# noahchalifour/rnnt-speech-recognition

Measured on AMD Instinct MI355X. Metric: rnnt_loss_grad_lattice_cells_per_sec, higher is better.
Workload: dtype f32

## Files before the change

rnnt-speech-recognition_amd/csrc/rnnt_common.h:

```cpp
#pragma once
#include <hip/hip_runtime.h>
#include <stdint.h>

#include <type_traits>

namespace rnnt {

constexpr float kNeg = -1.0e30f;
constexpr float kNegTest = -1.0e29f;
constexpr float kLog2e = 1.4426950408889634f;
constexpr float kLn2 = 0.6931471805599453f;
constexpr int kRebase = 8;

struct FastDiv {
    uint32_t d, m, s;
};
inline FastDiv make_fastdiv(uint32_t d) {
    FastDiv f;
    f.d = d;
    uint32_t s = 0;
    while ((1ull << s) < d) ++s;
    f.s = s;
    f.m = (uint32_t)((((1ull << s) - d) << 32) / d) + 1u;
    return f;
}
__device__ __forceinline__ uint32_t fdiv(uint32_t n, const FastDiv f) {
    return (__umulhi(n, f.m) + n) >> f.s;
}

struct TileGeom {
    int TT, UU, tiles_t, tiles_u, cpr;
    FastDiv div_tu, div_tt, divUU, div_cpr, divTT;
};

struct LossParams {
    const float *acts;
    float *grads;
    const int *labels;
    const int *label_lengths;
    const int *input_lengths;
    const float *cost_scale;
    float *costs;
    float *lse;
    float *W;
    float *A;
    float *Bt;
    float *offA;
    float *offB;
    double *ll;
    int *EA;
    int *EB;
    float *lik;
    int *flags;
    int NCl;
    float2 *pstat;
    int *lshift;
    int *bar;
    int nPstat;
    int pstatStride;
    int B, T, U, V, blank;
    int b0, nb;
    int visit_all;
    int precise;
    int N, Nr, Up, NC, NG;
    uint32_t cells;
    FastDiv divU, divT, divV, divOG;
    TileGeom tile;
};

struct WsLayout {
    size_t lse, W, A, Bt, offA, offB, ll, EA, EB, lik, flags, pstat, lshift, bar, total;
    int NCl, nPstat;
    int N, Nr, Up, NC, NG, OG;
};

inline size_t align_up(size_t x, size_t a) { return (x + a - 1) / a * a; }

constexpr int kMaxU = 8192;
inline int sweep_K(int U) {
    const int k = (U + 63) / 64;
    const int avail[] = {1, 2, 3, 4, 6, 8, 12, 16};
    for (int a : avail)
        if (k <= a) return a;
    return 0;
}
template <int K, int G>
struct SweepRing {
    static constexpr size_t kChunk = (size_t)G * 2 * 64 * K * sizeof(float);
    static constexpr int NB = (4 * kChunk + 16 <= 128 * 1024) ? 4 : 3;
    static constexpr size_t kBytes = NB * kChunk + 16;
    static_assert(kBytes <= 160 * 1024, "chunk ring exceeds the LDS");
};
template <typename F>
inline hipError_t sweep_dispatch(int U, F &&f) {
    using std::integral_constant;
    switch (sweep_K(U)) {
        case 1: return f(integral_constant<int, 1>(), integral_constant<int, 16>());
        case 2: return f(integral_constant<int, 2>(), integral_constant<int, 16>());
        case 3: return f(integral_constant<int, 3>(), integral_constant<int, 16>());
        case 4: return f(integral_constant<int, 4>(), integral_constant<int, 16>());
        case 6: return f(integral_constant<int, 6>(), integral_constant<int, 8>());
        case 8: return f(integral_constant<int, 8>(), integral_constant<int, 8>());
        case 12: return f(integral_constant<int, 12>(), integral_constant<int, 4>());
        case 16: return f(integral_constant<int, 16>(), integral_constant<int, 4>());
        default: return hipErrorInvalidValue;
    }
}
constexpr int kFillByte = 0xF1;

inline WsLayout make_layout(int T, int U, int B) {
    WsLayout w;
    w.N = T + U - 1;
    w.Nr = (int)align_up((size_t)w.N, 16);
    w.Up = sweep_K(U) ? 64 * sweep_K(U) : (int)align_up((size_t)U, 64);
    w.NC = w.Nr / kRebase + 1;
    w.OG = sweep_K(U) ? sweep_K(U) : 64;
    w.NG = w.Up / w.OG;
    size_t off = 0;
    auto take = [&](size_t bytes) {
        size_t o = off;
        off = align_up(off + bytes, 256);
        return o;
    };
    w.lse = take((size_t)B * T * U * sizeof(float));
    w.W = take((size_t)B * w.Nr * 2 * w.Up * sizeof(float));
    w.A = take((size_t)B * w.Nr * w.Up * sizeof(float));
    w.Bt = take((size_t)B * w.Nr * w.Up * sizeof(float));
    w.offA = take((size_t)B * w.NC * w.NG * sizeof(float));
    w.offB = take((size_t)B * w.NC * w.NG * sizeof(float));
    w.ll = take((size_t)B * 2 * sizeof(double));
    w.NCl = w.Nr / 4 + 1;
    w.EA = take((size_t)B * w.NCl * 64 * sizeof(int));
    w.EB = take((size_t)B * w.NCl * 64 * sizeof(int));
    w.lik = take((size_t)B * 4 * sizeof(float));
    w.flags = take((size_t)B * 4 * sizeof(int));
    {
        const int nu = (U + 31) / 32, UU = (U + nu - 1) / nu, TT = (256 / UU) > T ? T : (256 / UU);
        w.nPstat = ((T + TT - 1) / TT) * ((U + UU - 1) / UU) * 4;
    }
    w.pstat = take((size_t)B * w.nPstat * 2 * sizeof(float));
    w.lshift = take((size_t)B * sizeof(int));
    w.bar = take((size_t)B * 8 * sizeof(int));
    w.total = off;
    return w;
}

inline TileGeom make_tile(int T, int U, int V) {
    TileGeom g;
    const int nu = (U + 31) / 32;
    g.UU = (U + nu - 1) / nu;
    g.TT = 256 / g.UU;
    if (g.TT > T) g.TT = T;
    g.tiles_u = (U + g.UU - 1) / g.UU;
    g.tiles_t = (T + g.TT - 1) / g.TT;
    g.cpr = g.UU * V / 4;
    g.div_tu = make_fastdiv((uint32_t)g.tiles_u);
    g.div_tt = make_fastdiv((uint32_t)g.tiles_t);
    g.divUU = make_fastdiv((uint32_t)g.UU);
    g.divTT = make_fastdiv((uint32_t)(g.TT > 0 ? g.TT : 1));
    g.div_cpr = make_fastdiv((uint32_t)(g.cpr > 0 ? g.cpr : 1));
    return g;
}

constexpr float kExpTabLimit = 43.0f;
constexpr float kExpTab2Log2e = 2.8853900817779268f;
#ifdef __HIPCC__
__device__ __forceinline__ float exp_tab(float x) { return __builtin_amdgcn_exp2f(x * kExpTab2Log2e); }
__device__ __forceinline__ bool exp_tab_out_of_range(float x) { return !(fabsf(x) <= kExpTabLimit); }
#endif

constexpr int kHookBlocks = 1024;
struct JointHooks {
    int prep_mode;
    int prefilled;
    unsigned *dmax_enc;
    unsigned *dmax_pred;
};

#ifdef __HIPCC__
__device__ __forceinline__ void lds_dma16(const void *global, void *lds) {
    __builtin_amdgcn_global_load_lds((__attribute__((address_space(1))) const void *)global, (__attribute__((address_space(3))) void *)lds, 16, 0, 0);
}
#endif

inline int device_cu_count() {
    int dev = 0, n = 0;
    if (hipGetDevice(&dev) != hipSuccess) return 256;
    if (hipDeviceGetAttribute(&n, hipDeviceAttributeMultiprocessorCount, dev) != hipSuccess || n <= 0) return 256;
    return n;
}
template <typename Kernel>
inline hipError_t set_lds(Kernel kernel, size_t bytes) {
    if (bytes <= 64 * 1024) return hipSuccess;
    return hipFuncSetAttribute((const void *)kernel, hipFuncAttributeMaxDynamicSharedMemorySize, (int)bytes);
}

hipError_t launch_fill(void *dst, int byte, size_t bytes, hipStream_t s);
hipError_t launch_fill2(void *dst0, int byte0, size_t bytes0, void *dst1, int byte1, size_t bytes1, hipStream_t s);

bool tile_path_ok(const LossParams &p, bool grad);
hipError_t launch_lsm(const LossParams &p, hipStream_t s);
hipError_t launch_sweeps(const LossParams &p, hipStream_t s);
hipError_t launch_grad(const LossParams &p, hipStream_t s);
bool lin_path_ok(const LossParams &p);
hipError_t launch_lsm_lin(const LossParams &p, hipStream_t s);
hipError_t launch_sweeps_lin(const LossParams &p, hipStream_t s);
hipError_t launch_grad_lin(const LossParams &p, hipStream_t s);
hipError_t launch_redo_lin(const LossParams &p, bool force, hipStream_t s);

}
```

rnnt-speech-recognition_amd/csrc/rnnt_entrypoint.hip:

```cpp
#include "../../include/rnnt.h"
#include "rnnt_common.h"
#include "rnnt_lin.h"

using namespace rnnt;

namespace rnnt {
hipError_t joint_workspace_bytes(int T, int U, int B, int J, int V, int joint_dtype, size_t *bytes);
hipError_t joint_f16_backward_rows(void *workspace, int T, int U, int B, int J, int V, int rows[2], hipStream_t s);
hipError_t joint_backward_rows(void *workspace, int T, int U, int B, int J, int V, int rows[2], hipStream_t s);
hipError_t launch_joint_loss(const float *enc_proj, const float *pred_proj, const float *W2, const float *b2,
                             const int *labels, const int *label_lengths, const int *input_lengths,
                             const float *cost_scale, int J, int V, int B, int T, int U, int blank, float *costs,
                             float *d_enc_proj, float *d_pred_proj, float *dW2, float *db2, int joint_dtype,
                             int phases, void *workspace, hipStream_t s, const JointHooks *hooks);
hipError_t joint_aux_pointers(void *workspace, int T, int U, int B, int J, int V, float **expE, float **expP, float **tflag);
hipError_t launch_joint_prefill(void *workspace, int T, int U, int B, int J, int V, hipStream_t s);
bool joint_dtype_supported(int joint_dtype, int J, int V);
bool dense_supported(int H, int J);
hipError_t dense_workspace_bytes(int B, int T, int U, int H, int J, size_t base, size_t *bytes);
void dense_proj_pointers(void *workspace, int B, int T, int U, int H, int J, size_t base, float **enc_proj, float **pred_proj,
                         float **d_enc_proj, float **d_pred_proj);
void dense_hook_pointers(void *workspace, int B, int T, int U, int H, int J, size_t base, unsigned **dmax_enc, unsigned **dmax_pred);
hipError_t launch_dense_fwd(const float *enc, const float *pred, const float *W1, const float *b1, int B, int T, int U, int H, int J,
                            void *workspace, size_t base, float *expE, float *expP, float *tflag, hipStream_t s);
// ... 16 lines not shown
                             int T, int K, int joint_dtype, void *workspace, hipStream_t s);
hipError_t launch_beam_step(const float *pred_proj, int *parents, int *emitted, float *topk_logits, int *topk_symbols, float *lse,
                            int J, int V, int B, int T, int K, int N, int blank, int joint_dtype, void *workspace, hipStream_t s);
hipError_t launch_beam_results(int *hyps, int *hyp_lengths, float *scores, int *stable_lengths, int J, int V, int B, int T, int K,
                               int N, int joint_dtype, void *workspace, hipStream_t s);
hipError_t beam_stream_workspace_bytes(int Tc, int S, int K, int N, int H, int J, int V, int joint_dtype, size_t *bytes);
hipError_t launch_beam_stream_begin(const float *W1, const float *b1, const float *W2, const float *b2, int H, int J, int V, int S,
                                    int Tc, int K, int N, int joint_dtype, void *workspace, hipStream_t s);
hipError_t launch_beam_stream_feed(const float *enc, int Te, const int *chunk_frames, const int *reset, const int *final_, int H, int J,
                                   int V, int S, int Tc, int K, int N, int joint_dtype, void *workspace, hipStream_t s);
bool prednet_layout_ok(const rnntPrednetBlock *blocks, int L, int E, int V, int Jp, int R, size_t *bytes);
hipError_t launch_prednet_begin(const float *emb, const rnntPrednetBlock *blocks, int L, int E, int V, const float *W1, int Jp, int R,
                                float *out, void *workspace, hipStream_t s);
hipError_t launch_prednet_step(const int *emitted, const int *parents, float *out, const rnntPrednetBlock *blocks, int L, int E,
                               int V, int Jp, int R, void *workspace, hipStream_t s);
bool encoder_layout_ok(const rnntPrednetBlock *blocks, int L, int F, float bn_eps, int ridx, int f, int R, int Tmax, size_t *bytes);
hipError_t launch_encoder_begin(const rnntPrednetBlock *blocks, int L, int F, const float *bn_mean, const float *bn_var,
                                const float *bn_weight, const float *bn_bias, float bn_eps, int ridx, int f, int R, int Tmax,
                                void *workspace, hipStream_t s);
hipError_t launch_encoder_run(const float *x, int T, float *out, const rnntPrednetBlock *blocks, int L, int F, float bn_eps, int ridx,
                              int f, int R, int Tmax, void *workspace, hipStream_t s);
hipError_t launch_encoder_run_rows(const float *x, int T, const int *row_frames, const int *reset, float *out,
                                   const rnntPrednetBlock *blocks, int L, int F, float bn_eps, int ridx, int f, int R, int Tmax,
                                   void *workspace, hipStream_t s);
bool lstm_train_layout_ok(int R, int T, int H, int P, bool proj, size_t *bytes);
hipError_t launch_lstm_train_fwd(float *gates, const float *W_hh, const float *W_hr, float *y, float *c, float *h, int R, int T, int H,
                                 int P, void *workspace, hipStream_t s);
hipError_t launch_lstm_train_bwd(float *gates, const float *c, const float *dy, const float *W_hh, const float *W_hr, float *dr, int R,
                                 int T, int H, int P, void *workspace, hipStream_t s);
hipError_t launch_prednet_reset(const int *reset, float *out, const rnntPrednetBlock *blocks, int L, int E, int V, int Jp, int R,
                                void *workspace, hipStream_t s);
hipError_t greedy_stream_workspace_bytes(int Tc, int S, int H, int J, int V, int joint_dtype, size_t *bytes);
hipError_t launch_greedy_stream_begin(const float *W1, const float *b1, const float *W2, const float *b2, int H, int J, int V, int S,
                                      int Tc, int joint_dtype, void *workspace, hipStream_t s);
hipError_t launch_greedy_stream_feed(const float *enc, int Te, const int *chunk_frames, const int *reset, const int *final_,
                                     const int *max_symbols, int max_per_frame, int *hyp_lengths, float *scores, int *all_done, int H,
                                     int J, int V, int S, int Tc, int joint_dtype, void *workspace, hipStream_t s);
}

static rnntStatus_t check_options(const rnntOptions &o) {
    if (o.loc != RNNT_GPU) return RNNT_STATUS_INVALID_VALUE;
    if (!o.batch_first) return RNNT_STATUS_INVALID_VALUE;
    if (o.maxT <= 0 || o.maxU <= 0 || o.blank_label < 0) return RNNT_STATUS_INVALID_VALUE;
    if (o.maxU > kMaxU) return RNNT_STATUS_INVALID_VALUE;
    return RNNT_STATUS_SUCCESS;
}

static bool fill_params(LossParams &p, const float *acts, float *grads, const int *labels,
                        const int *label_lengths, const int *input_lengths, const float *cost_scale, int V,
                        int B, float *costs, void *workspace, const rnntOptions &o) {
    const long long cells = (long long)B * o.maxT * o.maxU;
    if (cells <= 0 || cells >= (1ll << 31)) return false;
    if (((uintptr_t)workspace & 255) != 0) return false;
    const WsLayout w = make_layout(o.maxT, o.maxU, B);
    char *ws = (char *)workspace;
    p.acts = acts;
    p.grads = grads;
    p.labels = labels;
    p.label_lengths = label_lengths;
    p.input_lengths = input_lengths;
    p.cost_scale = cost_scale;
    p.costs = costs;
    p.lse = (float *)(ws + w.lse);
    p.W = (float *)(ws + w.W);
    p.A = (float *)(ws + w.A);
    p.Bt = (float *)(ws + w.Bt);
    p.offA = (float *)(ws + w.offA);
    p.offB = (float *)(ws + w.offB);
    p.ll = (double *)(ws + w.ll);
    p.EA = (int *)(ws + w.EA);
    p.EB = (int *)(ws + w.EB);
    p.lik = (float *)(ws + w.lik);
    p.flags = (int *)(ws + w.flags);
    p.NCl = w.NCl;
    p.pstat = (float2 *)(ws + w.pstat);
    p.lshift = (int *)(ws + w.lshift);
    p.bar = (int *)(ws + w.bar);
    p.nPstat = w.nPstat;
    p.pstatStride = 4;
    p.B = B, p.T = o.maxT, p.U = o.maxU, p.V = V, p.blank = o.blank_label;
    p.b0 = 0, p.nb = B;
    p.precise = 0;
    p.visit_all = 0;
    p.tile = make_tile(o.maxT, o.maxU, V);
    p.N = w.N, p.Nr = w.Nr, p.Up = w.Up, p.NC = w.NC, p.NG = w.NG;
    p.cells = (uint32_t)cells;
    p.divU = make_fastdiv((uint32_t)o.maxU);
    p.divT = make_fastdiv((uint32_t)o.maxT);
    p.divV = make_fastdiv((uint32_t)V);
    p.divOG = make_fastdiv((uint32_t)w.OG);
    return true;
}

namespace rnnt {
bool fill_loss_params(LossParams &p, const float *acts, float *grads, const int *labels, const int *label_lengths,
                      const int *input_lengths, const float *cost_scale, int V, int B, float *costs, void *workspace,
                      int maxT, int maxU, int blank) {
    rnntOptions o;
    o.loc = RNNT_GPU, o.stream = nullptr, o.blank_label = blank, o.maxT = maxT, o.maxU = maxU, o.batch_first = true;
    return fill_params(p, acts, grads, labels, label_lengths, input_lengths, cost_scale, V, B, costs, workspace, o);
}
}

static rnntStatus_t from_hip(hipError_t e) {
    if (e == hipSuccess) return RNNT_STATUS_SUCCESS;
    if (e == hipErrorInvalidValue) return RNNT_STATUS_INVALID_VALUE;
    return RNNT_STATUS_EXECUTION_FAILED;
}

extern "C" {

int get_warprnnt_version(void) { return 1; }

const char *rnntGetStatusString(rnntStatus_t status) {
    switch (status) {
        case RNNT_STATUS_SUCCESS: return "no error";
        case RNNT_STATUS_MEMOPS_FAILED: return "hip memcpy or memset failed";
        case RNNT_STATUS_INVALID_VALUE: return "invalid value";
        case RNNT_STATUS_EXECUTION_FAILED: return "execution failed";
        case RNNT_STATUS_UNKNOWN_ERROR:
        default: return "unknown error";
    }
}

rnntStatus_t get_workspace_size(int maxT, int maxU, int minibatch, bool gpu, size_t *size_bytes) {
    if (!size_bytes || maxT <= 0 || maxU <= 0 || minibatch <= 0 || !gpu) return RNNT_STATUS_INVALID_VALUE;
    *size_bytes = make_layout(maxT, maxU, minibatch).total;
    return RNNT_STATUS_SUCCESS;
}

static rnntStatus_t run_forward(LossParams &p, const WsLayout &w, hipStream_t s) {
    if (lin_path_ok(p)) {
        hipError_t e = launch_lsm_lin(p, s);
        if (e != hipSuccess) return from_hip(e);
        return from_hip(launch_sweeps_lin(p, s));
    }
    if (!tile_path_ok(p, false) && launch_fill(p.W, kFillByte, w.A - w.W, s) != hipSuccess) return RNNT_STATUS_MEMOPS_FAILED;
    p.precise = 1;
    hipError_t e = launch_lsm(p, s);
    if (e != hipSuccess) return from_hip(e);
    return from_hip(launch_sweeps(p, s));
}

static rnntStatus_t validate(const void *acts, const void *labels, const void *ll, const void *il, const void *ws,
                      int V, int B, const rnntOptions &o) {
    if (!acts || !labels || !ll || !il || !ws) return RNNT_STATUS_INVALID_VALUE;
    if (V <= 0 || B <= 0) return RNNT_STATUS_INVALID_VALUE;
    rnntStatus_t st = check_options(o);
    if (st != RNNT_STATUS_SUCCESS) return st;
    if (o.blank_label >= V) return RNNT_STATUS_INVALID_VALUE;
    return RNNT_STATUS_SUCCESS;
}

rnntStatus_t compute_rnnt_loss_fwd(const float *acts, const int *flat_labels, const int *label_lengths,
                                   const int *input_lengths, int alphabet_size, int minibatch, float *costs,
                                   void *workspace, rnntOptions options) {
    if (!costs) return RNNT_STATUS_INVALID_VALUE;
    rnntStatus_t st = validate(acts, flat_labels, label_lengths, input_lengths, workspace, alphabet_size, minibatch,
                               options);
    if (st != RNNT_STATUS_SUCCESS) return st;
    LossParams p;
    if (!fill_params(p, acts, nullptr, flat_labels, label_lengths, input_lengths, nullptr, alphabet_size,
                     minibatch, costs, workspace, options))
        return RNNT_STATUS_INVALID_VALUE;
    hipStream_t s = (hipStream_t)options.stream;
    const WsLayout w = make_layout(options.maxT, options.maxU, minibatch);
    st = run_forward(p, w, s);
    if (st != RNNT_STATUS_SUCCESS || !lin_path_ok(p)) return st;
    return from_hip(launch_redo_lin(p, false, s));
}

static rnntStatus_t run_backward(LossParams &p, hipStream_t s) {
    if (!lin_path_ok(p)) return from_hip(launch_grad(p, s));
    const bool patch = tile_path_ok(p, true);
    if (patch) {
        hipError_t e = launch_grad_lin(p, s);
        if (e != hipSuccess) return from_hip(e);
    }
    return from_hip(launch_redo_lin(p, !patch, s));
}

rnntStatus_t compute_rnnt_loss_bwd(const float *acts, float *grads, const int *flat_labels,
                                   const int *label_lengths, const int *input_lengths, const float *cost_scale,
                                   int alphabet_size, int minibatch, void *workspace, rnntOptions options) {
    if (!grads) return RNNT_STATUS_INVALID_VALUE;
    rnntStatus_t st = validate(acts, flat_labels, label_lengths, input_lengths, workspace, alphabet_size, minibatch,
                               options);
    if (st != RNNT_STATUS_SUCCESS) return st;
    LossParams p;
    if (!fill_params(p, acts, grads, flat_labels, label_lengths, input_lengths, cost_scale, alphabet_size,
                     minibatch, nullptr, workspace, options))
        return RNNT_STATUS_INVALID_VALUE;
    return run_backward(p, (hipStream_t)options.stream);
}

rnntStatus_t compute_rnnt_loss_flags(const float *acts, float *grads, const int *flat_labels,
                                     const int *label_lengths, const int *input_lengths, const float *cost_scale,
                                     int alphabet_size, int minibatch, float *costs, void *workspace,
                                     rnntOptions options, unsigned int flags) {
    if (flags & ~(unsigned)RNNT_VISIT_ALL) return RNNT_STATUS_INVALID_VALUE;
    if (!grads)
        return compute_rnnt_loss_fwd(acts, flat_labels, label_lengths, input_lengths, alphabet_size, minibatch,
                                     costs, workspace, options);
    rnntStatus_t st = validate(acts, flat_labels, label_lengths, input_lengths, workspace, alphabet_size, minibatch,
                               options);
    if (st != RNNT_STATUS_SUCCESS) return st;
    LossParams p;
    if (!fill_params(p, acts, grads, flat_labels, label_lengths, input_lengths, cost_scale, alphabet_size,
                     minibatch, costs, workspace, options))
        return RNNT_STATUS_INVALID_VALUE;
    p.visit_all = (flags & RNNT_VISIT_ALL) ? 1 : 0;
    hipStream_t s = (hipStream_t)options.stream;
    if (costs) {
        const WsLayout w = make_layout(options.maxT, options.maxU, minibatch);
        st = run_forward(p, w, s);
        if (st != RNNT_STATUS_SUCCESS) return st;
    }
    return run_backward(p, s);
}

rnntStatus_t compute_rnnt_loss_ex(const float *acts, float *grads, const int *flat_labels,
                                  const int *label_lengths, const int *input_lengths, const float *cost_scale,
                                  int alphabet_size, int minibatch, float *costs, void *workspace,
                                  rnntOptions options) {
    if (grads && !costs) return RNNT_STATUS_INVALID_VALUE;
    return compute_rnnt_loss_flags(acts, grads, flat_labels, label_lengths, input_lengths, cost_scale, alphabet_size, minibatch,
                                   costs, workspace, options, 0u);
}

rnntStatus_t compute_rnnt_loss(const float *acts, float *grads, const int *flat_labels,
                               const int *label_lengths, const int *input_lengths, int alphabet_size,
                               int minibatch, float *costs, void *workspace, rnntOptions options) {
    return compute_rnnt_loss_ex(acts, grads, flat_labels, label_lengths, input_lengths, nullptr, alphabet_size,
                                minibatch, costs, workspace, options);
}

rnntStatus_t get_joint_workspace_size(int maxT, int maxU, int minibatch, int joint_size, int alphabet_size,
                                      size_t *size_bytes) {
    if (!size_bytes || maxT <= 0 || maxU <= 0 || minibatch <= 0 || joint_size <= 0 || alphabet_size <= 0)
        return RNNT_STATUS_INVALID_VALUE;
    return from_hip(joint_workspace_bytes(maxT, maxU, minibatch, joint_size, alphabet_size, -1, size_bytes));
}

static rnntStatus_t joint_call(const float *enc_proj, const float *pred_proj, const float *W2, const float *b2,
                               const int *flat_labels, const int *label_lengths, const int *input_lengths,
                               const float *cost_scale, int joint_size, int alphabet_size, int minibatch, float *costs,
                               float *d_enc_proj, float *d_pred_proj, float *dW2, float *db2, int joint_dtype,
                               int phases, void *workspace, const rnntOptions &options) {
    if (!enc_proj || !pred_proj || !W2 || !b2 || !flat_labels || !label_lengths || !input_lengths || !workspace)
        return RNNT_STATUS_INVALID_VALUE;
    if ((phases & 1) && !costs) return RNNT_STATUS_INVALID_VALUE;
    if (joint_size <= 0 || alphabet_size <= 0 || minibatch <= 0) return RNNT_STATUS_INVALID_VALUE;
    rnntStatus_t st = check_options(options);
    if (st != RNNT_STATUS_SUCCESS) return st;
    if (options.blank_label >= alphabet_size) return RNNT_STATUS_INVALID_VALUE;
    if (options.maxU > 1024) return RNNT_STATUS_INVALID_VALUE;
    if (joint_dtype & ~(0xff | RNNT_VISIT_ALL)) return RNNT_STATUS_INVALID_VALUE;
    if (joint_dtype & RNNT_VISIT_ALL) phases |= 8;
    joint_dtype &= 0xff;
    if (!joint_dtype_supported(joint_dtype, joint_size, alphabet_size)) return RNNT_STATUS_INVALID_VALUE;
    const bool any_grad = d_enc_proj || d_pred_proj || dW2 || db2;
    if (any_grad && !(d_enc_proj && d_pred_proj && dW2 && db2)) return RNNT_STATUS_INVALID_VALUE;
    if ((phases & 2) && !(phases & 1) && !any_grad) return RNNT_STATUS_INVALID_VALUE;
    return from_hip(launch_joint_loss(enc_proj, pred_proj, W2, b2, flat_labels, label_lengths, input_lengths,
                                      cost_scale, joint_size, alphabet_size, minibatch, options.maxT, options.maxU,
                                      options.blank_label, costs, d_enc_proj, d_pred_proj, dW2, db2, joint_dtype,
                                      phases, workspace, (hipStream_t)options.stream, nullptr));
}

rnntStatus_t compute_rnnt_joint_loss(const float *enc_proj, const float *pred_proj, const float *W2,
                                     const float *b2, const int *flat_labels, const int *label_lengths,
                                     const int *input_lengths, const float *cost_scale, int joint_size,
                                     int alphabet_size, int minibatch, float *costs, float *d_enc_proj,
                                     float *d_pred_proj, float *dW2, float *db2, int joint_dtype, void *workspace,
                                     rnntOptions options) {
    return joint_call(enc_proj, pred_proj, W2, b2, flat_labels, label_lengths, input_lengths, cost_scale, joint_size,
                      alphabet_size, minibatch, costs, d_enc_proj, d_pred_proj, dW2, db2, joint_dtype, 3, workspace,
                      options);
}

rnntStatus_t compute_rnnt_joint_loss_fwd(const float *enc_proj, const float *pred_proj, const float *W2,
                                         const float *b2, const int *flat_labels, const int *label_lengths,
                                         const int *input_lengths, int joint_size, int alphabet_size, int minibatch,
                                         float *costs, int joint_dtype, void *workspace, rnntOptions options) {
    return joint_call(enc_proj, pred_proj, W2, b2, flat_labels, label_lengths, input_lengths, nullptr, joint_size,
                      alphabet_size, minibatch, costs, nullptr, nullptr, nullptr, nullptr, joint_dtype, 1 | 4, workspace,
                      options);
}

rnntStatus_t compute_rnnt_joint_loss_bwd(const float *enc_proj, const float *pred_proj, const float *W2,
                                         const float *b2, const int *flat_labels, const int *label_lengths,
                                         const int *input_lengths, const float *cost_scale, int joint_size,
                                         int alphabet_size, int minibatch, float *d_enc_proj, float *d_pred_proj,
                                         float *dW2, float *db2, int joint_dtype, void *workspace,
                                         rnntOptions options) {
// ... 544 lines not shown
```

rnnt-speech-recognition_amd/csrc/rnnt_kernels.hip:

```cpp
#include "rnnt_common.h"
#include "rnnt_cell.h"
#include "rnnt_sweep.h"
#include "rnnt_cellwave.h"
#include "rnnt_lin.h"
#include "rnnt_cellbody.h"

#include <float.h>
#include <math.h>
#include <stdlib.h>

namespace rnnt {


typedef float gs_v4f __attribute__((ext_vector_type(4)));
__device__ __forceinline__ void grad_store16(gs_v4f *dst, const gs_v4f v) { __builtin_nontemporal_store(v, dst); }

constexpr int kFillRows = 16;

template <int VP, bool GRAD, bool AL = true, bool LIN = false>
__global__ __launch_bounds__(256) void cell_tile_kernel(const LossParams p) {
    extern __shared__ __attribute__((aligned(16))) float lds[];
    const int tid = threadIdx.x;
    const int lane = tid & 63;
    const int wave = __builtin_amdgcn_readfirstlane(tid >> 6);
    const int V = p.V;
    const TileGeom &tg = p.tile;
    const uint32_t n_patch_wg = (uint32_t)p.nb * (uint32_t)tg.tiles_t * (uint32_t)tg.tiles_u;
    uint32_t vblock = blockIdx.x;
    if (!GRAD) {
        const uint32_t per = (uint32_t)p.Nr / kFillRows, n_fill = (uint32_t)p.nb * per;
        const uint32_t pgs = (n_patch_wg + 7u) >> 3, fgs = (n_fill + 7u) >> 3, P = (pgs + fgs) / fgs;
        const uint32_t g = blockIdx.x >> 3, l8 = blockIdx.x & 7u;
        const uint32_t k = g / P;
        const bool is_fill = g - k * P == P - 1u && k < fgs;
        if (is_fill) {
            const uint32_t f = k * 8u + l8;
            if (f >= n_fill) return;
            const int fb = p.b0 + (int)(f / per), chunk = (int)(f % per);
            const int Tf = length_T(p, fb), Uf = length_U(p, fb);
            const int Nf = Tf + Uf - 1;
            float2 *Wb = (float2 *)p.W + (size_t)fb * p.Nr * p.Up;
            const float2 z = LIN ? make_float2(0.f, 0.f) : make_float2(kNeg, kNeg);
            for (int idx = tid; idx < kFillRows * p.Up; idx += 256) {
                const int rr = idx / p.Up, u = idx - rr * p.Up;
                const int n = chunk * kFillRows + rr;
                if (n < Nf && (u < max(0, n - Tf + 1) || u > min(n, Uf - 1))) Wb[(size_t)n * p.Up + u] = z;
            }
            return;
        }
        vblock = (g - min(k, fgs)) * 8u + l8;
        if (vblock >= n_patch_wg) return;
    }
    uint32_t bid;
    {
        const uint32_t nwg = n_patch_wg, xcd = vblock & 7u, idx = vblock >> 3;
        const uint32_t q = nwg >> 3, r = nwg & 7u;
        bid = (xcd < r ? xcd * (q + 1u) : r * (q + 1u) + (xcd - r) * q) + idx;
        if (GRAD) bid = (xcd < r ? xcd * (q + 1u) : r * (q + 1u) + (xcd - r) * q) + ((xcd < r ? q + 1u : q) - 1u - idx);
    }
    const uint32_t q1 = fdiv(bid, tg.div_tu);
    const uint32_t tu = bid - q1 * (uint32_t)tg.tiles_u;
    const uint32_t bb = fdiv(q1, tg.div_tt);
    const uint32_t tt = q1 - bb * (uint32_t)tg.tiles_t;
    const int b = p.b0 + (int)bb;
    const int t0 = (int)tt * tg.TT, u0 = (int)tu * tg.UU;
    const int Tb = length_T(p, b), Ub = length_U(p, b);
    if (GRAD && LIN && lin_skip(p, b)) return;

    const int rows_valid = max(0, min(tg.TT, Tb - t0));
    const int cols_valid = max(0, min(tg.UU, Ub - u0));
    const int rows_in = max(0, min(tg.TT, p.T - t0));
    const int cols_in = max(0, min(tg.UU, p.U - u0));
    const int q_valid = cols_valid * V / 4;
    const int q_in = cols_in * V / 4;
    const int row_lds = AL ? tg.UU * V : ((tg.UU * V + 3 + 3) & ~3);
    const size_t row_f = (size_t)p.U * V;
    const size_t patch0 = ((size_t)(b * p.T + t0) * p.U + u0) * V;

    auto store_row = [&](const int r, const float *src) {
        const size_t s0 = patch0 + r * row_f;
        if (AL) {
            for (int q = lane; q < q_in; q += 64) {
                typedef float v4f __attribute__((ext_vector_type(4)));
                const v4f v = src ? ((const v4f *)src)[q] : (v4f){0.f, 0.f, 0.f, 0.f};
                grad_store16((v4f *)(p.grads + s0 + q * 4), v);
            }
        } else {
            const int a = (int)(s0 & 3), len = cols_in * V;
            float *base = p.grads + (s0 - a);
            for (int q = lane; q * 4 < a + len; q += 64) {
                const int e0 = q * 4 - a;
                typedef float v4f __attribute__((ext_vector_type(4)));
                const v4f vv = src ? ((const v4f *)src)[q] : (v4f){0.f, 0.f, 0.f, 0.f};
                const float v[4] = {vv[0], vv[1], vv[2], vv[3]};
                if (e0 >= 0 && e0 + 3 < len) {
                    grad_store16((v4f *)(base + q * 4), vv);
                } else {
#pragma unroll
                    for (int k = 0; k < 4; ++k)
                        if (e0 + k >= 0 && e0 + k < len) base[q * 4 + k] = v[k];
                }
            }
        }
    };

    float2 *const pslot = p.pstat + (size_t)b * p.nPstat + ((size_t)tt * tg.tiles_u + tu) * 4 + wave;
    if (rows_valid == 0 || cols_valid == 0) {
        if (GRAD) {
            for (int r = wave; r < rows_in; r += 4) store_row(r, nullptr);
        }
        if (!GRAD && LIN && lane == 0) *pslot = make_float2(0.f, 0.f);
        return;
    }

    const uint32_t r = fdiv((uint32_t)tid, tg.divUU);
    const int cu = tid - (int)r * tg.UU;
    Cell cl;
    cl.b = b, cl.t = t0 + (int)r, cl.u = u0 + cu, cl.Tb = Tb, cl.Ub = Ub;
    cl.valid = ((int)r < rows_valid) && (cu < cols_valid);
    const uint32_t c = ((uint32_t)(b * p.T + cl.t)) * (uint32_t)p.U + (uint32_t)cl.u;

    LinGrad lg = {};
    uint32_t lword = ~0u;
    if (GRAD && LIN) {
        bool live = false;
        if (cl.valid) {
            lg = lin_grad_setup(p, cl);
            if (lg.bad) atomicOr(p.flags + 4 * cl.b + kFlagG, 1);
            live = p.visit_all || !(lg.l2occ <= (float)-kOccFloorWave);
            cl.valid = live;
        }
        const uint64_t m = __ballot(live);
        const int ncell = tg.TT * tg.UU, nw = (ncell + 31) >> 5;
        uint32_t *const lw = (uint32_t *)lds;
        if (lane == 0 && wave * 64 < ncell) lw[2 * wave] = (uint32_t)m;
        if (lane == 0 && wave * 64 + 32 < ncell) lw[2 * wave + 1] = (uint32_t)(m >> 32);
        __syncthreads();
        lword = lane < nw ? lw[lane] : 0u;
        __syncthreads();
        if (__ballot(lword != 0u) == 0) {
            for (int rr = wave; rr < rows_in; rr += 4) store_row(rr, nullptr);
            return;
        }
    }
    auto cells_live = [&](const int klo, const int khi) -> bool {
        const uint32_t wlo = (uint32_t)__shfl((int)lword, klo >> 5), whi = (uint32_t)__shfl((int)lword, khi >> 5);
        const uint64_t bits = ((uint64_t)whi << 32 | wlo) >> (klo & 31);
        return (bits & ((2ull << (khi - klo)) - 1ull)) != 0;
    };

    for (int r = wave; r < rows_valid; r += 4) {
        const size_t s0 = patch0 + r * row_f;
        const int a = AL ? 0 : (int)(s0 & 3);
        const float *src = p.acts + (s0 - a);
        float *dst = lds + r * row_lds;
        const int nq = AL ? q_valid : (a + cols_valid * V + 3) / 4;
        for (int q0 = 0; q0 < nq; q0 += 64) {
            const int q = q0 + lane;
            bool need = q < nq;
            if (GRAD && LIN) {
                const int e = min(q, nq - 1) * 4 - a;
                const int lo = (int)fdiv((uint32_t)max(0, e), p.divV), hi = AL ? lo : (int)fdiv((uint32_t)min(e + 3, cols_valid * V - 1), p.divV);
                need = cells_live(r * tg.UU + lo, r * tg.UU + hi) && need;
            }
            if (need) {
                __builtin_amdgcn_global_load_lds((glb_void *)(src + q * 4), (lds_void *)(dst + q0 * 4), 16, 0, 0);
            }
        }
    }
    wait_vm0();
    __syncthreads();

    float stat = 0.f;
    if (AL) {
        if ((GRAD && tid < tg.TT * tg.UU) || cl.valid) stat = cell_body<VP, true, GRAD, LIN>(p, cl, c, lds + tid * V, lds + tid * V, &lg);
    } else if ((int)r < tg.TT) {
        const int a = (int)((patch0 + r * row_f) & 3);
        if (GRAD || cl.valid) stat = cell_body<VP, false, GRAD, LIN>(p, cl, c, lds + r * row_lds + a + cu * V, lds + r * row_lds + a + cu * V, &lg);
    }
    if (!GRAD && LIN) {
        float cnt = cl.valid ? 1.f : 0.f;
        stat = cl.valid ? stat : 0.f;
#pragma unroll
        for (int off = 32; off > 0; off >>= 1) stat += __shfl_xor(stat, off), cnt += __shfl_xor(cnt, off);
        if (lane == 0) *pslot = make_float2(stat, cnt);
        __syncthreads();
        float2 *const Wp = (float2 *)p.W + ((size_t)b * p.Nr + t0 + u0) * p.Up + u0;
        const uint32_t total = (uint32_t)(tg.TT + tg.UU - 1) * (uint32_t)tg.TT;
        for (uint32_t j = tid; j < total; j += 256) {
            const uint32_t d = fdiv(j, tg.divTT);
            const int rr = (int)(j - d * (uint32_t)tg.TT), cc = (int)d - rr;
            if (rr < rows_valid && cc >= 0 && cc < cols_valid) {
                float2 v;
                if (AL) {
                    v = *(const float2 *)(lds + (rr * tg.UU + cc) * V);
                } else {
                    const float *src = lds + rr * row_lds + (int)((patch0 + rr * row_f) & 3) + cc * V;
                    v = make_float2(src[0], src[1]);
                }
                Wp[(size_t)(rr + cc) * p.Up + cc] = v;
            }
        }
    }
    if (GRAD && !AL) {
        __syncthreads();
        for (int rr = wave; rr < rows_in; rr += 4) store_row(rr, lds + rr * row_lds);
    } else if (GRAD) {
        __syncthreads();
        for (int rr = wave; rr < rows_in; rr += 4) {
            const float4 *srcl = (const float4 *)(lds + rr * row_lds);
            float *dstg = p.grads + patch0 + rr * row_f;
            for (int q = lane; q < q_in; q += 64) {
                typedef float v4f __attribute__((ext_vector_type(4)));
                grad_store16((v4f *)(dstg + q * 4), ((const v4f *)srcl)[q]);
            }
        }
    }
}

template <bool V4, bool GRAD>
__global__ __launch_bounds__(256) void cell_wave_kernel(const LossParams p) {
    const uint32_t cpw = (uint32_t)wave_cells(p.V);
    const uint32_t c_lo = (blockIdx.x * 4u + (threadIdx.x >> 6)) * cpw;
    cell_wave_range<V4, GRAD>(p, c_lo, min(c_lo + cpw, p.cells), threadIdx.x & 63);
}

__device__ __forceinline__ void fill_span(uint32_t *dst, const uint32_t word, const size_t nwords, const unsigned blk) {
    if ((((uintptr_t)dst) & 15) == 0) {
        const size_t n4 = nwords >> 2;
        const uint4 q = make_uint4(word, word, word, word);
        const size_t base = (size_t)blk * 1024 + threadIdx.x;
#pragma unroll
        for (int k = 0; k < 4; ++k)
            if (base + 256 * k < n4) ((uint4 *)dst)[base + 256 * k] = q;
        if (blk == 0 && threadIdx.x < (nwords & 3)) dst[n4 * 4 + threadIdx.x] = word;
    } else {
        const size_t base = (size_t)blk * 4096 + threadIdx.x;
#pragma unroll
        for (int k = 0; k < 16; ++k)
            if (base + 256 * k < nwords) dst[base + 256 * k] = word;
    }
}
__global__ __launch_bounds__(256) void fill_kernel(uint32_t *dst, const uint32_t word, const size_t nwords) {
    fill_span(dst, word, nwords, blockIdx.x);
}
__global__ __launch_bounds__(256) void fill2_kernel(uint32_t *dst0, const uint32_t word0, const size_t nwords0, const unsigned grid0,
                                                    uint32_t *dst1, const uint32_t word1, const size_t nwords1) {
    if (blockIdx.x < grid0)
        fill_span(dst0, word0, nwords0, blockIdx.x);
    else
        fill_span(dst1, word1, nwords1, blockIdx.x - grid0);
}

static inline uint32_t fill_word(int byte) {
    const uint32_t b = (uint32_t)(byte & 0xff);
    return b | (b << 8) | (b << 16) | (b << 24);
}

hipError_t launch_fill(void *dst, int byte, size_t bytes, hipStream_t s) {
    if (bytes == 0) return hipSuccess;
    if ((bytes & 3) != 0 || (((uintptr_t)dst) & 3) != 0) return hipErrorInvalidValue;
    const size_t nwords = bytes >> 2;
    const size_t grid = (nwords + 4095) / 4096;
    if (grid > 0x7fffffffu) return hipErrorInvalidValue;
    hipLaunchKernelGGL(fill_kernel, dim3((unsigned)grid), dim3(256), 0, s, (uint32_t *)dst, fill_word(byte), nwords);
    return hipGetLastError();
}

hipError_t launch_fill2(void *dst0, int byte0, size_t bytes0, void *dst1, int byte1, size_t bytes1, hipStream_t s) {
    if (bytes0 == 0) return launch_fill(dst1, byte1, bytes1, s);
    if (bytes1 == 0) return launch_fill(dst0, byte0, bytes0, s);
    if (((bytes0 | bytes1) & 3) != 0 || ((((uintptr_t)dst0) | ((uintptr_t)dst1)) & 3) != 0) return hipErrorInvalidValue;
    const size_t n0 = bytes0 >> 2, n1 = bytes1 >> 2;
    const size_t g0 = (n0 + 4095) / 4096, g1 = (n1 + 4095) / 4096;
    if (g0 + g1 > 0x7fffffffu) return hipErrorInvalidValue;
    hipLaunchKernelGGL(fill2_kernel, dim3((unsigned)(g0 + g1)), dim3(256), 0, s, (uint32_t *)dst0, fill_word(byte0), n0, (unsigned)g0,
                       (uint32_t *)dst1, fill_word(byte1), n1);
    return hipGetLastError();
}

bool tile_path_ok(const LossParams &p, bool grad) {
    if (p.V > 60) return false;
    if ((p.V % 4) != 0 && (((size_t)p.cells * (size_t)p.V) % 4) != 0) return false;
    if (((uintptr_t)p.acts & 15) != 0) return false;
    if (grad && ((uintptr_t)p.grads & 15) != 0) return false;
    return true;
}

template <bool GRAD, bool LIN = false>
static hipError_t launch_cell(const LossParams &p, hipStream_t s) {
    if (LIN && !tile_path_ok(p, GRAD)) return hipErrorInvalidValue;
    if (tile_path_ok(p, GRAD)) {
        const unsigned n_patch = (unsigned)p.nb * p.tile.tiles_t * p.tile.tiles_u;
        unsigned blocks = n_patch;
        if (!GRAD)
            blocks = (((n_patch + 7u) >> 3) + (((unsigned)p.nb * (unsigned)(p.Nr / kFillRows) + 7u) >> 3)) * 8u;
        const size_t shm = (size_t)p.tile.TT * p.tile.UU * p.V * sizeof(float);
// ... 184 lines not shown
```

rnnt-speech-recognition_amd/csrc/rnnt_lin_kernels.hip:

```cpp
#include "rnnt_common.h"
#include "rnnt_cell.h"
#include "rnnt_sweep.h"
#include "rnnt_cellwave.h"
#include "rnnt_lin.h"
#include "rnnt_cellbody.h"
#include "rnnt_redo.h"

namespace rnnt {

__device__ __forceinline__ float dpp_lower_zero(float x) {
    return __int_as_float(__builtin_amdgcn_update_dpp(0, __float_as_int(x), 0x138 , 0xf, 0xf, true));
}
__device__ __forceinline__ float dpp_upper_zero(float x) {
    return __int_as_float(__builtin_amdgcn_update_dpp(0, __float_as_int(x), 0x130 , 0xf, 0xf, true));
}
__device__ __forceinline__ int dpp_lower_i(int x, int fill) {
    return __builtin_amdgcn_update_dpp(fill, x, 0x138, 0xf, 0xf, false);
}
__device__ __forceinline__ int dpp_upper_i(int x, int fill) {
    return __builtin_amdgcn_update_dpp(fill, x, 0x130, 0xf, 0xf, false);
}

struct LinState {
    int E;
// ... 238 lines not shown
            lin_issue_row<K, 1>(wq[1], abase);
            lin_alpha_fast_steps<K, G, SH, 0>(a, wq, abase, st, voff, lane, r0);
        } else {
            for (int i = 0; i < G; ++i) {
                const int n = r0 + i + 1;
                if (n > last_row) break;
                LinRow<K> wc;
                lin_load_row<K>(wc, cur + i * 2 * Up);
                lin_alpha_step<K>(a, wc, st.d);
                if ((n & ((1 << SH) - 1)) == 0) lin_renorm<K, false, SH>(a, st, n >> SH);
                store_diag<K, false>(st.row, voff, lane, a);
                st.row += Up;
            }
        }
        if (ck + 1 < nchunks) {
            asm volatile("s_waitcnt lgkmcnt(0)" ::: "memory");
            if (lane == 0) lds_post(lk.consumed, ck + 1);
        }
    }
    {
        const float *wrow = bufs + ((nchunks - 1) % NB) * chunkf + (last_row % G) * 2 * Up + 2 * u0;
#pragma unroll
        for (int j = 0; j < K; ++j)
            if (u0 + j == Ub - 1) lin_record(p, b, 0, a[j] * wrow[2 * j], st.E, timed_out);
    }
}

template <int K, int G, int NB, int SH>
__device__ void lin_beta_sweep(const LossParams &p, float *bufs, const LdLink lk, const int b, const int lane) {
    constexpr int Up = 64 * K, chunkf = G * 2 * Up;
    const int Tb = length_T(p, b), Ub = length_U(p, b);
    const int Nb = Tb + Ub - 1;
    float *out = p.Bt + (size_t)b * p.Nr * Up;
    const int voff = lane * K * 4;
    const int u0 = lane * K;

    float bv[K];
#pragma unroll
    for (int j = 0; j < K; ++j) bv[j] = (u0 + j == Ub - 1) ? 1.f : 0.f;
    const int last = Nb - 1;
    const int ckl = last / G;
    LinState st;
    st.E = 0, st.d = 0;
    st.tab = p.EB + (size_t)b * p.NCl * 64 + lane;
    st.row = out + (size_t)last * Up;

    LandedView lv;
    lv.addr0 = lk.landed;
#pragma unroll
    for (int w = 0; w < kLinLoaders; ++w) lv.have[w] = 0;
    bool timed_out = lengths_invalid(p, b);
    for (int ck = ckl; ck >= 0; --ck) {
        const int i_ring = ckl - ck;
        timed_out |= !lv.wait(i_ring);
        const float *cur = bufs + (i_ring % NB) * chunkf + 2 * u0;
        const int r0 = ck * G;
        if (r0 + G - 1 < last) {
            const uint32_t abase = (uint32_t)(uintptr_t)((lds_void *)cur);
            LinRow<K> wq[3];
            lin_issue_row<K, G - 1>(wq[0], abase);
            lin_issue_row<K, G - 2>(wq[1], abase);
            lin_beta_fast_steps<K, G, SH, 0>(bv, wq, abase, st, voff, lane, r0);
        } else {
            for (int ii = 0; ii < G; ++ii) {
                const int i = G - 1 - ii;
                const int n = r0 + i;
                if (n > last) continue;
                LinRow<K> wc;
                lin_load_row<K>(wc, cur + i * 2 * Up);
                lin_beta_step<K>(bv, wc, st.d);
                if ((n & ((1 << SH) - 1)) == (1 << SH) - 1 || n == last) lin_renorm<K, true, SH>(bv, st, n >> SH);
                store_diag<K, false>(st.row, voff, lane, bv);
                st.row -= Up;
            }
        }
        if (ck > 0) {
            asm volatile("s_waitcnt lgkmcnt(0)" ::: "memory");
            if (lane == 0) lds_post(lk.consumed, i_ring + 1);
        }
    }
    if (lane == 0) lin_record(p, b, 1, bv[0], st.E, timed_out);
}

template <int K, int G, int NB>
__global__ __launch_bounds__(64 * (1 + kLinLoaders)) void lin_sweep_kernel(const LossParams p) {
    extern __shared__ __attribute__((aligned(16))) float lds[];
    constexpr int chunkf = G * 2 * 64 * K;
    const int tid = threadIdx.x, lane = tid & 63;
    const int wave = __builtin_amdgcn_readfirstlane(tid >> 6);
    const int b = p.b0 + (int)(blockIdx.x >> 1);
    const bool beta = (blockIdx.x & 1) != 0;
    int *ctr = (int *)(lds + NB * chunkf);
    if (tid < 2 * kLinLoaders) ctr[tid] = 0;
    __syncthreads();
    LdLink lk;
    lk.landed = (uint32_t)(uintptr_t)((lds_void *)ctr);
    lk.consumed = lk.landed + 4u;
    if (wave >= 1) {
        LdLink mine = lk;
        mine.landed = lk.landed + 8u * (uint32_t)(wave - 1);
        if (beta)
            sweep_loader<K, G, NB, true, kLinLoaders>(p, lds, mine, b, lane, wave - 1);
        else
            sweep_loader<K, G, NB, false, kLinLoaders>(p, lds, mine, b, lane, wave - 1);
    } else {
        constexpr int SHmax = lin_shift_max(K);
        int sh = SHmax;
        if constexpr (SHmax > 2) {
            float sum = 0.f, cnt = 0.f;
            const float2 *ps = p.pstat + (size_t)b * p.nPstat;
            const int stride = p.pstatStride, npatch = p.nPstat / stride;
            for (int i0 = 0; i0 < npatch; i0 += 512) {
                float2 q[8];
#pragma unroll
                for (int k = 0; k < 8; ++k) {
                    const int i = i0 + 64 * k + lane;
                    q[k] = (i < npatch) ? ps[(size_t)stride * i] : make_float2(0.f, 0.f);
                }
#pragma unroll
                for (int k = 0; k < 8; ++k) sum += q[k].x, cnt += q[k].y;
            }
#pragma unroll
            for (int off = 32; off > 0; off >>= 1) sum += __shfl_xor(sum, off), cnt += __shfl_xor(cnt, off);
            sh = (sum > kLinDecayBits * cnt) ? 2 : SHmax;
            sh = __builtin_amdgcn_readfirstlane(sh);
        }
        if constexpr (SHmax > 2) {
            if (sh == 2) {
                if (beta)
                    lin_beta_sweep<K, G, NB, 2>(p, lds, lk, b, lane);
                else
                    lin_alpha_sweep<K, G, NB, 2>(p, lds, lk, b, lane);
                return;
            }
        }
        if (beta)
            lin_beta_sweep<K, G, NB, SHmax>(p, lds, lk, b, lane);
        else
            lin_alpha_sweep<K, G, NB, SHmax>(p, lds, lk, b, lane);
    }
}

template <int K, int G, int NB>
__global__ __launch_bounds__(kRedoThreads) void lin_redo_kernel(const LossParams p, const int force, const int team) {
    extern __shared__ __attribute__((aligned(16))) float lds[];
    constexpr int chunkf = G * 2 * 64 * K;
    const int tid = threadIdx.x;
    const int ub = (int)blockIdx.x / team;
    const int b = p.b0 + ub;
    RedoTeam tm;
    tm.k = (int)blockIdx.x - ub * team, tm.n = team, tm.bar = p.bar + kRedoCtr * b, tm.ok = true;
    int *fl = p.flags + 4 * b;
    typedef int i32x4 __attribute__((ext_vector_type(4)));
    typedef double f64x2 __attribute__((ext_vector_type(2)));
    const i32x4 fw = __builtin_nontemporal_load((const i32x4 *)fl);
    const f64x2 lw = __builtin_nontemporal_load((const f64x2 *)(p.ll + 2 * b));
    const int state = fw[kFlagState];
    bool redo = false;
    if (state != 2) {
        const bool agree = fabs(lw[0] - lw[1]) * 0.6931471805599453 <= 2e-5 + 1e-8 * fabs(lw[0]);
        redo = force || (fw[kFlagA] | fw[kFlagB] | fw[kFlagG]) != 0 || !agree;
        if (!redo) return;
    } else if (!p.grads) {
        return;
    }
    if (redo) redo_lattice<K, G, NB>(p, b, tm, lds, tid);
    uint32_t lo, hi;
    redo_cell_range(p, b, tm, lo, hi);
    if (p.grads) redo_cells<true>(p, lo, hi, tid, lds, NB * chunkf);
    if (!tm.ok) {
        if (p.costs && tm.k == 0 && tid == 0) st_f32_wt(p.costs + b, NAN);
        if (p.grads)
            for (size_t i = (size_t)lo * p.V + tid; i < (size_t)hi * p.V; i += kRedoThreads) p.grads[i] = NAN;
    }
}

bool lin_path_ok(const LossParams &p) { return p.V >= 2 && sweep_K(p.U) >= 1 && tile_path_ok(p, false); }

template <int K, int G>
static hipError_t launch_lin_sweep(const LossParams &p, hipStream_t s) {
    using R = SweepRing<K, G>;
    static_assert(2 * kLinLoaders * sizeof(int) <= 16, "the loaders' flag words exceed the ring's 16 bytes");
    hipError_t e = set_lds(lin_sweep_kernel<K, G, R::NB>, R::kBytes);
    if (e != hipSuccess) return e;
    hipLaunchKernelGGL((lin_sweep_kernel<K, G, R::NB>), dim3(2 * p.nb), dim3(64 * (1 + kLinLoaders)), R::kBytes, s, p);
    return hipGetLastError();
}
template <int K, int G>
static hipError_t launch_lin_redo(const LossParams &p, const bool force, hipStream_t s) {
    using R = SweepRing<K, G>;
    hipError_t e = set_lds(lin_redo_kernel<K, G, R::NB>, R::kBytes);
    if (e != hipSuccess) return e;
    const int team = redo_team_size(p.nb, p.T, p.U, device_cu_count());
    hipLaunchKernelGGL((lin_redo_kernel<K, G, R::NB>), dim3(p.nb * team), dim3(kRedoThreads), R::kBytes, s, p, force ? 1 : 0, team);
    return hipGetLastError();
}

hipError_t launch_sweeps_lin(const LossParams &p, hipStream_t s) {
    return sweep_dispatch(p.U, [&](auto K, auto G) { return launch_lin_sweep<K, G>(p, s); });
}
hipError_t launch_redo_lin(const LossParams &p, const bool force, hipStream_t s) {
    return sweep_dispatch(p.U, [&](auto K, auto G) { return launch_lin_redo<K, G>(p, force, s); });
}

}
```

Before: 14.04 billion.

## Zero-fill gradients on idle CUs during sweeps and skip dead-cell stores

When the batch leaves most CUs idle during the alpha/beta sweep, extra blocks appended to the sweep launch zero the whole gradient buffer in parallel with the serial sweeps. The later gradient kernel then skips stores for tiles and 16-byte segments whose cells are all dead, since they are already zero. This moves write traffic off the critical path into otherwise unused CU time. It costs extra launch blocks, added per-store liveness checks, and the risk that a partially masked segment leaves stale values if the liveness mapping is off.

```diff
diff --git a/rnnt-speech-recognition_amd/csrc/rnnt_common.h b/rnnt-speech-recognition_amd/csrc/rnnt_common.h
--- a/rnnt-speech-recognition_amd/csrc/rnnt_common.h
+++ b/rnnt-speech-recognition_amd/csrc/rnnt_common.h
@@ -61,6 +61,8 @@
     int B, T, U, V, blank;
     int b0, nb;
     int visit_all;
+    int grads_zeroed;
+    uint32_t fill_span;
     int precise;
     int N, Nr, Up, NC, NG;
     uint32_t cells;
@@ -181,6 +183,8 @@
 __device__ __forceinline__ void lds_dma16(const void *global, void *lds) {
     __builtin_amdgcn_global_load_lds((__attribute__((address_space(1))) const void *)global, (__attribute__((address_space(3))) void *)lds, 16, 0, 0);
 }
+typedef float gs_v4f __attribute__((ext_vector_type(4)));
+__device__ __forceinline__ void grad_store16(gs_v4f *dst, const gs_v4f v) { __builtin_nontemporal_store(v, dst); }
 #endif
 
 inline int device_cu_count() {
@@ -203,6 +207,7 @@
 hipError_t launch_sweeps(const LossParams &p, hipStream_t s);
 hipError_t launch_grad(const LossParams &p, hipStream_t s);
 bool lin_path_ok(const LossParams &p);
+bool lin_prefill_ok(const LossParams &p);
 hipError_t launch_lsm_lin(const LossParams &p, hipStream_t s);
 hipError_t launch_sweeps_lin(const LossParams &p, hipStream_t s);
 hipError_t launch_grad_lin(const LossParams &p, hipStream_t s);
diff --git a/rnnt-speech-recognition_amd/csrc/rnnt_entrypoint.hip b/rnnt-speech-recognition_amd/csrc/rnnt_entrypoint.hip
--- a/rnnt-speech-recognition_amd/csrc/rnnt_entrypoint.hip
+++ b/rnnt-speech-recognition_amd/csrc/rnnt_entrypoint.hip
@@ -122,6 +122,7 @@
     p.b0 = 0, p.nb = B;
     p.precise = 0;
     p.visit_all = 0;
+    p.grads_zeroed = 0, p.fill_span = 0;
     p.tile = make_tile(o.maxT, o.maxU, V);
     p.N = w.N, p.Nr = w.Nr, p.Up = w.Up, p.NC = w.NC, p.NG = w.NG;
     p.cells = (uint32_t)cells;
@@ -251,6 +252,7 @@
         return RNNT_STATUS_INVALID_VALUE;
     p.visit_all = (flags & RNNT_VISIT_ALL) ? 1 : 0;
     hipStream_t s = (hipStream_t)options.stream;
+    p.grads_zeroed = (costs && !p.visit_all && lin_prefill_ok(p)) ? 1 : 0;
     if (costs) {
         const WsLayout w = make_layout(options.maxT, options.maxU, minibatch);
         st = run_forward(p, w, s);
diff --git a/rnnt-speech-recognition_amd/csrc/rnnt_kernels.hip b/rnnt-speech-recognition_amd/csrc/rnnt_kernels.hip
--- a/rnnt-speech-recognition_amd/csrc/rnnt_kernels.hip
+++ b/rnnt-speech-recognition_amd/csrc/rnnt_kernels.hip
@@ -12,8 +12,6 @@
 namespace rnnt {
 
 
-typedef float gs_v4f __attribute__((ext_vector_type(4)));
-__device__ __forceinline__ void grad_store16(gs_v4f *dst, const gs_v4f v) { __builtin_nontemporal_store(v, dst); }
 
 constexpr int kFillRows = 16;
 
@@ -104,9 +102,11 @@
         }
     };
 
+    const bool zeroed = GRAD && LIN && AL && p.grads_zeroed != 0;
+
     float2 *const pslot = p.pstat + (size_t)b * p.nPstat + ((size_t)tt * tg.tiles_u + tu) * 4 + wave;
     if (rows_valid == 0 || cols_valid == 0) {
-        if (GRAD) {
+        if (GRAD && !zeroed) {
             for (int r = wave; r < rows_in; r += 4) store_row(r, nullptr);
         }
         if (!GRAD && LIN && lane == 0) *pslot = make_float2(0.f, 0.f);
@@ -139,7 +139,8 @@
         lword = lane < nw ? lw[lane] : 0u;
         __syncthreads();
         if (__ballot(lword != 0u) == 0) {
-            for (int rr = wave; rr < rows_in; rr += 4) store_row(rr, nullptr);
+            if (!zeroed)
+                for (int rr = wave; rr < rows_in; rr += 4) store_row(rr, nullptr);
             return;
         }
     }
@@ -210,9 +211,18 @@
         for (int rr = wave; rr < rows_in; rr += 4) {
             const float4 *srcl = (const float4 *)(lds + rr * row_lds);
             float *dstg = p.grads + patch0 + rr * row_f;
-            for (int q = lane; q < q_in; q += 64) {
-                typedef float v4f __attribute__((ext_vector_type(4)));
-                grad_store16((v4f *)(dstg + q * 4), ((const v4f *)srcl)[q]);
+            typedef float v4f __attribute__((ext_vector_type(4)));
+            if (zeroed) {
+                const int c16 = (int)(((uintptr_t)dstg >> 4) & 7u);
+                for (int q0 = 0; q0 < q_in; q0 += 64) {
+                    const int q = min(q0 + lane, q_in - 1);
+                    const int ls = ((q + c16) & ~7) - c16;
+                    const int lo = (int)fdiv((uint32_t)(max(ls, 0) * 4), p.divV), hi = (int)fdiv((uint32_t)(min(ls + 7, q_in - 1) * 4 + 3), p.divV);
+                    const bool need = cells_live(rr * tg.UU + lo, rr * tg.UU + hi);
+                    if (need && q0 + lane < q_in) grad_store16((v4f *)(dstg + q * 4), ((const v4f *)srcl)[q]);
+                }
+            } else {
+                for (int q = lane; q < q_in; q += 64) grad_store16((v4f *)(dstg + q * 4), ((const v4f *)srcl)[q]);
             }
         }
     }
diff --git a/rnnt-speech-recognition_amd/csrc/rnnt_lin_kernels.hip b/rnnt-speech-recognition_amd/csrc/rnnt_lin_kernels.hip
--- a/rnnt-speech-recognition_amd/csrc/rnnt_lin_kernels.hip
+++ b/rnnt-speech-recognition_amd/csrc/rnnt_lin_kernels.hip
@@ -344,10 +344,42 @@
     if (lane == 0) lin_record(p, b, 1, bv[0], st.E, timed_out);
 }
 
-template <int K, int G, int NB>
+constexpr int kFillFlight = 8;
+constexpr size_t kFillTrip = 64 * (1 + kLinLoaders) * kFillFlight;
+__host__ __device__ inline size_t fill_head_words(const float *dst, const size_t nwords) {
+    const size_t h = (size_t)((0u - (unsigned)((uintptr_t)dst >> 2)) & 3u);
+    return h < nwords ? h : nwords;
+}
+__device__ __forceinline__ void lin_fill_zeros(float *dst, const size_t nwords, const unsigned k, const size_t per) {
+    constexpr size_t kThreads = 64 * (1 + kLinLoaders), kTrip = kFillTrip;
+    const unsigned tid = threadIdx.x;
+    const size_t head = fill_head_words(dst, nwords);
+    const size_t n4 = (nwords - head) >> 2, tail = (nwords - head) & 3;
+    if (k == 0) {
+        if (tid < head) dst[tid] = 0.f;
+        if (tid < tail) dst[head + 4 * n4 + tid] = 0.f;
+    }
+    gs_v4f *const body = (gs_v4f *)(dst + head);
+    const size_t lo = min(n4, (size_t)k * per), hi = min(n4, lo + per);
+    const gs_v4f z = {0.f, 0.f, 0.f, 0.f};
+    for (size_t i = lo + tid; i < hi; i += kTrip) {
+#pragma unroll
+        for (int j = 0; j < kFillFlight; ++j)
+            if (i + kThreads * j < hi) grad_store16(body + i + kThreads * j, z);
+    }
+}
+
+template <int K, int G, int NB, bool FILL = false>
 __global__ __launch_bounds__(64 * (1 + kLinLoaders)) void lin_sweep_kernel(const LossParams p) {
     extern __shared__ __attribute__((aligned(16))) float lds[];
     constexpr int chunkf = G * 2 * 64 * K;
+    if constexpr (FILL) {
+        const unsigned nsw = 2u * (unsigned)p.nb;
+        if (blockIdx.x >= nsw) {
+            lin_fill_zeros(p.grads, (size_t)p.cells * (size_t)p.V, blockIdx.x - nsw, (size_t)p.fill_span);
+            return;
+        }
+    }
     const int tid = threadIdx.x, lane = tid & 63;
     const int wave = __builtin_amdgcn_readfirstlane(tid >> 6);
     const int b = p.b0 + (int)(blockIdx.x >> 1);
@@ -439,10 +471,25 @@
 
 bool lin_path_ok(const LossParams &p) { return p.V >= 2 && sweep_K(p.U) >= 1 && tile_path_ok(p, false); }
 
+static int lin_fill_groups(const int nb) { return device_cu_count() - 2 * nb; }
+bool lin_prefill_ok(const LossParams &p) {
+    return p.grads && lin_path_ok(p) && tile_path_ok(p, true) && (p.V % 4) == 0 && 2 * lin_fill_groups(p.nb) >= device_cu_count();
+}
+
 template <int K, int G>
 static hipError_t launch_lin_sweep(const LossParams &p, hipStream_t s) {
     using R = SweepRing<K, G>;
     static_assert(2 * kLinLoaders * sizeof(int) <= 16, "the loaders' flag words exceed the ring's 16 bytes");
+    if (p.grads_zeroed) {
+        const int n_fill = lin_fill_groups(p.nb);
+        const size_t nwords = (size_t)p.cells * (size_t)p.V, n4 = (nwords - fill_head_words(p.grads, nwords)) >> 2;
+        LossParams q = p;
+        q.fill_span = (uint32_t)(((n4 + n_fill - 1) / n_fill + kFillTrip - 1) / kFillTrip * kFillTrip);
+        hipError_t e = set_lds(lin_sweep_kernel<K, G, R::NB, true>, R::kBytes);
+        if (e != hipSuccess) return e;
+        hipLaunchKernelGGL((lin_sweep_kernel<K, G, R::NB, true>), dim3(2 * p.nb + n_fill), dim3(64 * (1 + kLinLoaders)), R::kBytes, s, q);
+        return hipGetLastError();
+    }
     hipError_t e = set_lds(lin_sweep_kernel<K, G, R::NB>, R::kBytes);
     if (e != hipSuccess) return e;
     hipLaunchKernelGGL((lin_sweep_kernel<K, G, R::NB>), dim3(2 * p.nb), dim3(64 * (1 + kLinLoaders)), R::kBytes, s, p);
```

New measurement: 12.39 billion. -11.8%, worse.
